# hpc4cmb/flacarray

Measured on AMD Instinct MI355X. Metric: Msamples/s encode+decode, 4096ch x 1Msamp int32, higher is better.
Workload: dtype int32

## Files before the change

### flacarray_amd/csrc/encode_fused.hpp

```cpp
#pragma once
#include "encode_kernels.hpp"
#include "quantize_kernels.hpp"

namespace fa {

constexpr int kFSmpWords = 65 * 32;
#ifndef FA_F_SCANW
#define FA_F_SCANW 4
#endif
#ifndef FA_F_RING
#define FA_F_RING 1024
#endif
constexpr int kFRingWords = FA_F_RING;
constexpr int kFRingMask = kFRingWords - 1;
constexpr int kFRingBlocks = kFRingWords / 64;
constexpr int kFRowBlocks = 12;
static_assert(kFRingBlocks - kFRowBlocks - 1 >= 1, "the ring must hold the longest row and a partial block beside what waits to be flushed");
constexpr int kFWaveWords = kFSmpWords + kFRingWords + 4 + 16;
constexpr int kFWaves = 4;
constexpr int kFCrcSlice = 1024;
constexpr int kFCrcXpow = 520;
#ifndef FA_F_SLEEP
#define FA_F_SLEEP 8
#endif
#ifndef FA_F_WBATCH
#define FA_F_WBATCH 4
#endif
#ifndef FA_F_CEIL
#define FA_F_CEIL 1
#endif
#ifndef FA_F_BFLY_N
#define FA_F_BFLY_N 1
#endif
#ifndef FA_F_SHLEV
#define FA_F_SHLEV 1
#endif
#ifndef FA_F_SHLEV_MAXMLO
#define FA_F_SHLEV_MAXMLO 12
#endif
#ifndef FA_F_SHPOLL
#define FA_F_SHPOLL 256
#endif
#ifndef FA_F_SHSLEEP
#define FA_F_SHSLEEP 4
#endif
#ifndef FA_F_PARKN
#define FA_F_PARKN 32
#endif
#ifndef FA_F_PARKBLK
#define FA_F_PARKBLK 1
#endif
#ifndef FA_F_PARK
#define FA_F_PARK 1
#endif
// ... 12 lines not shown
    double escale_full;
    const float* win;
    const uint4* hdr;
    uint8_t* blob;
    int64_t capacity;
    int64_t hb;
    uint32_t* frame_bytes;
    int64_t* frame_abs;
    FrameInfo* info;
    uint32_t* ticket;
    uint32_t* size_pub;
    unsigned long long* off_pub;
    int64_t* total;
    int* err;
    const uint16_t* crc_tab;
    unsigned long long* stamps;
    int64_t* starts;
    int64_t* nbytes;
};

__device__ __forceinline__ int fsmp_unit(int c1, int u) { return 32 * c1 + 4 * (u ^ (c1 & 7)); }
__device__ __forceinline__ int fsmp_idx(int s) {
    const int c1 = (s >> 5) + 1;
    return fsmp_unit(c1, (s >> 2) & 7) + (s & 3);
}

__device__ __forceinline__ int lane_id_opaque() {
    int l;
    asm volatile("v_mbcnt_lo_u32_b32 %0, -1, 0\n\tv_mbcnt_hi_u32_b32 %0, -1, %0" : "=v"(l));
    return l;
}
__device__ __forceinline__ int rice_fold(int r) { return (int)(((uint32_t)r << 1) ^ (uint32_t)(r >> 31)); }
__device__ __forceinline__ int dpp_wave_shr1(int old, int v) { return __builtin_amdgcn_update_dpp(old, v, 0x138, 0xF, 0xF, false); }

__device__ __forceinline__ uint16_t crc16_mulmod(uint16_t a, uint16_t b) {
    uint32_t r = 0;
#pragma unroll
    for (int i = 15; i >= 0; --i) {
        r = (r << 1) ^ ((r & 0x8000u) ? 0x18005u : 0u);
        if ((b >> i) & 1) r ^= a;
    }
    return (uint16_t)r;
}

template <typename T>
__device__ __forceinline__ T lb_load(const T* p) { return __hip_atomic_load(p, __ATOMIC_RELAXED, __HIP_MEMORY_SCOPE_AGENT); }

struct SplitRiceSearch {
    int pred_order, pmax, lane;
    uint32_t TA, TB, S, n, pb, SC, best;
    int M, p, k, bpo, kb;
    bool slot;
    __device__ __forceinline__ void start(uint32_t ta, uint32_t tb, int pred_order_, int pmax_, int lane_) {
        pred_order = pred_order_; pmax = pmax_; lane = lane_;
        TA = wave_incl_scan_u32(ta);
        TB = wave_incl_scan_u32(tb);
    }
    __device__ __forceinline__ void gather() {
        M = (2 << pmax) - 1;
        const int Lp = M - lane;
        slot = (Lp >= 1);
        const int po = slot ? (31 - __clz(Lp)) : 0;
        p = lane - (M + 1 - (2 << po));
        const uint32_t psz = 4096u >> po;
        const int cpp = 128 >> po;
        const bool inB = (po > 0) && (p >= (1 << (po - 1)));
// ... 996 lines not shown
        a.info[g].shift = (int32_t)(uint32_t)__builtin_amdgcn_s_memrealtime();
        __builtin_amdgcn_s_waitcnt(0);
    }
#endif
    if (lane_w == 0) {
        __hip_atomic_store(a.size_pub + gu, 0x80000000u | total_bytes, __ATOMIC_RELAXED, __HIP_MEMORY_SCOPE_AGENT);
        a.frame_bytes[g] = total_bytes;
    }
    (void)F;
#ifndef FA_TIMELINE
    if (lane_w == 0 && a.info) {
        FrameInfo fi;
        fi.type = type;
        fi.order = (type >= 2) ? order : 0;
        fi.porder = (type >= 2) ? porder : 0;
        fi.wasted = wasted;
        fi.shift = (type == 3) ? shift : 0;
        fi.precision = (type == 3) ? precision : 0;
        fi.nbytes = (int32_t)total_bytes;
        fi.blocksize = bs;
        a.info[g] = fi;
    }
#endif

#ifdef FA_F_ANALYSIS_ONLY
    if (lane_w == 0) a.frame_abs[g] = g * (int64_t)kSlotBytes + (s + 1) * a.hb;
    return;
#endif
    kpar[lane_w] = (uint8_t)kbest;
    for (int i = lane_w; i < kFRingWords; i += 64) ring[i] = 0;
    if (lane_w == 0) ring[kFRingWords] = 0;
    lds_fence();
    uint32_t pos = 0;
    uint32_t blocks_flushed = 0;
    uint8_t* dst = nullptr;
    bool dropped = false, have_dst = false;
    uint32_t crc_t = 0;

    auto put_bits = [&](uint32_t P, uint32_t val, uint32_t nb) __attribute__((always_inline)) {
        const uint32_t off = P & 31u;
        const uint64_t X = (uint64_t)val << (64u - nb - off);
        const uint32_t a0 = (P >> 3) & (uint32_t)(4 * kFRingWords - 4);
        atomicOr(reinterpret_cast<uint32_t*>(reinterpret_cast<char*>(ring) + a0), (uint32_t)(X >> 32));
        atomicOr(reinterpret_cast<uint32_t*>(reinterpret_cast<char*>(ring) + a0 + 4), (uint32_t)X);
    };
    auto put_code = [&](uint32_t P, uint32_t u, uint32_t shl) __attribute__((always_inline)) {
        const uint32_t vL = (u << shl) | 0x80000000u;
        uint32_t wi;
        asm("v_bfe_u32 %0, %1, 5, %2" : "=v"(wi) : "v"(P), "n"(__builtin_ctz((unsigned)kFRingWords)));
        uint32_t* const w = ring + wi;
        atomicOr(w, __builtin_amdgcn_alignbit(0u, vL, P));
        atomicOr(w + 1, __builtin_amdgcn_alignbit(vL, 0u, P));
    };
    unsigned long long off_word = 0;
    auto lb_issue = [&]() __attribute__((always_inline)) {
#ifndef FA_F_NOLB
        off_word = lb_load(a.off_pub + gu);
#endif
    };
    auto lb_resolve = [&]() __attribute__((always_inline)) {
        uint32_t spins = 0;
        bool fail = false;
#ifdef FA_TIMELINE
        const uint32_t tl_req_ = (uint32_t)__builtin_amdgcn_s_memrealtime();
#endif
#ifdef FA_F_NOLB
        off_word = (unsigned long long)(g * (int64_t)kSlotBytes + (s + 1) * a.hb);
#else
        while (off_word == 0) {
            __builtin_amdgcn_s_sleep(FA_F_SLEEP);
            if (++spins > kLbSpinLimit) { fail = true; break; }
            off_word = lb_load(a.off_pub + gu);
        }
#endif
#ifdef FA_TIMELINE
        if (lane_w == 0 && a.info) {
            a.info[g].precision = (int32_t)tl_req_;
            a.info[g].blocksize = (int32_t)(uint32_t)__builtin_amdgcn_s_memrealtime();
        }
#endif
#ifdef FA_STAMPS
        st_[3] += spins;
#endif
        const int64_t off = (int64_t)(((uint64_t)(uint32_t)__builtin_amdgcn_readfirstlane((int)(uint32_t)(off_word >> 32)) << 32) |
                                      (uint32_t)__builtin_amdgcn_readfirstlane((int)(uint32_t)off_word));
        fail = __builtin_amdgcn_readfirstlane((int)fail) != 0;
        if (fail || off < 0 || off + (int64_t)total_bytes > a.capacity) {
            if (lane_w == 0) atomicOr(a.err, fail ? 2 : 1);
            dropped = true;
        } else {
            dst = a.blob + off;
            if (lane_w == 0) a.frame_abs[g] = off;
        }
        have_dst = true;
    };
    auto crc_word = [&](uint32_t wv) __attribute__((always_inline)) {
        const uint32_t w = wv ^ (crc_t << 16);
        const uint32_t t0 = crc_s[w >> 24], t1 = crc_s[256 + ((w >> 16) & 255u)], t2 = crc_s[512 + ((w >> 8) & 255u)], t3 = crc_s[768 + (w & 255u)];
        uint32_t x01;
        asm("v_xor_b32 %0, %1, %2" : "=v"(x01) : "v"(t0), "v"(t1));
        asm("v_bitop3_b32 %0, %1, %2, %3 bitop3:0x96" : "=v"(crc_t) : "v"(x01), "v"(t2), "v"(t3));
    };
    uint32_t carry = 0;
    auto emit_word = [&](uint32_t m, uint32_t Q) __attribute__((always_inline)) {
        const uint32_t sh = (uint32_t)(reinterpret_cast<uintptr_t>(dst) & 3u);
        const uint32_t P = (uint32_t)dpp_wave_shr1((int)carry, (int)Q);
        carry = (uint32_t)__builtin_amdgcn_readlane((int)Q, 63);
        const uint32_t V = __builtin_amdgcn_alignbit(P, Q, 8u * sh);
        const int lo = (int)(4u * m) - (int)sh;
        if (lo >= 0 && (uint32_t)lo + 4u <= total_bytes) {
            *reinterpret_cast<uint32_t*>(dst + lo) = __builtin_bswap32(V);
        } else {
#pragma unroll
            for (int i = 0; i < 4; ++i) {
                const int b = lo + i;
                if (b >= 0 && (uint32_t)b < total_bytes) dst[b] = (uint8_t)(V >> (24 - 8 * i));
            }
        }
    };
    auto emit_block = [&](uint32_t blk, uint32_t Q) __attribute__((always_inline)) {
        const uint32_t sh = (uint32_t)(reinterpret_cast<uintptr_t>(dst) & 3u);
        const uint32_t P = (uint32_t)dpp_wave_shr1((int)carry, (int)Q);
        carry = (uint32_t)__builtin_amdgcn_readlane((int)Q, 63);
        const uint32_t V = __builtin_amdgcn_alignbit(P, Q, 8u * sh);
        *reinterpret_cast<uint32_t*>(dst - sh + 256u * blk + 4u * (uint32_t)lane_w) = __builtin_bswap32(V);
    };
#if FA_F_PARKBLK
    uint32_t park[FA_F_PARKN];
#endif
    uint32_t n_parked = 0;
    auto take_block = [&](uint32_t blk) __attribute__((always_inline)) {
        const uint32_t wi = (blk * 64 + lane_w) & kFRingMask;
        uint32_t wv = ring[wi];
        ring[wi] = 0;
        if (__builtin_expect((blk & (uint32_t)(kFRingBlocks - 1)) == 0, 0)) {
            if (lane_w == 0) { wv |= ring[kFRingWords]; ring[kFRingWords] = 0; }
        }
        return wv;
    };
    auto flush_blocks = [&](uint32_t row_bits, bool final_call) __attribute__((always_inline)) {
        const uint32_t done = (uint32_t)__builtin_amdgcn_readfirstlane((int)(pos >> 11));
        blocks_flushed = (uint32_t)__builtin_amdgcn_readfirstlane((int)blocks_flushed);
        const uint32_t hi_blk = (uint32_t)__builtin_amdgcn_readfirstlane((int)((pos + row_bits) >> 11));
        if (!final_call && hi_blk - blocks_flushed < (uint32_t)kFRingBlocks) return;
#ifdef FA_STAMPS
        const unsigned long long tq0_ = fa_memtime();
#endif
        if (!have_dst) {
#if FA_F_PARKBLK
            if (!final_call && off_word == 0) {
                off_word = lb_load(a.off_pub + gu);
                n_parked = (uint32_t)__builtin_amdgcn_readfirstlane((int)n_parked);
                while (blocks_flushed < done && n_parked < (uint32_t)FA_F_PARKN) {
                    const uint32_t wv = take_block(blocks_flushed);
                    crc_word(wv);
                    park[n_parked] = wv;
                    n_parked++;
                    blocks_flushed++;
                }
                if (hi_blk - blocks_flushed < (uint32_t)kFRingBlocks) {
#ifdef FA_STAMPS
                    st_[14] += fa_memtime() - tq0_;
#endif
                    return;
                }
            }
#endif
            lb_resolve();
        }
#ifdef FA_STAMPS
        st_[14] += fa_memtime() - tq0_;
#endif
#if FA_F_PARKBLK
        n_parked = (uint32_t)__builtin_amdgcn_readfirstlane((int)n_parked);
        if (__builtin_expect(n_parked != 0, 0)) {
            if (!dropped) {
                emit_word((uint32_t)lane_w, park[0]);
                for (uint32_t i = 1; i < n_parked; ++i) emit_block(i, park[i]);
            }
            n_parked = 0;
        }
#endif
        if (__builtin_expect(blocks_flushed == 0 && done > 0, 0)) {
            const uint32_t wv = take_block(0);
            crc_word(wv);
            if (!dropped) emit_word((uint32_t)lane_w, wv);
            blocks_flushed = 1;
            __builtin_amdgcn_sched_barrier(0);
        }
        while (blocks_flushed < done) {
            const uint32_t wv = take_block(blocks_flushed);
            crc_word(wv);
            if (!dropped) emit_block(blocks_flushed, wv);
            blocks_flushed++;
        }
    };

#if FA_F_PARKBLK
#pragma unroll
    for (int i = 0; i < FA_F_PARKN; ++i) asm volatile("" : "=v"(park[i]));
#endif
    lb_issue();
    {
        const int tc = (type == 0) ? 0x00 : (type == 1) ? 0x01 : (type == 2) ? (0x08 | order) : (0x20 | (order - 1));
        const uint32_t smask = (bps == 32) ? 0xffffffffu : ((1u << bps) - 1u);
        const int nwarm = (type == 0) ? 1 : (type >= 2) ? order : 0;
        constexpr int kWarmLanes = (MLO > 4) ? MLO : 4;
        constexpr int kL_warm = 6, kL_lpc = kL_warm + kWarmLanes, kL_coef = kL_lpc + 1, kL_rice = kL_coef + MLO;
        static_assert(kL_rice < 64, "preamble fields must fit the wave");
        uint32_t fv = 0, fnb = 0;
        if (lane_w == 0) { fv = fhe.x; fnb = 32; }
        else if (lane_w == 1) { fv = fhe.y; fnb = (fhe.w >> 8) & 0xFFu; }
        else if (lane_w == 2) { fv = fhe.z & 0xFFFFu; fnb = (fhe.w >> 16) & 0xFFu; }
        else if (lane_w == 3) { fv = fhe.z >> 16; fnb = fhe.w >> 24; }
        else if (lane_w == 4) { fv = ((fhe.w & 0xFFu) << 8) | (uint32_t)((tc << 1) | (wasted ? 1 : 0)); fnb = 16; }
        else if (lane_w == 5) { if (wasted) { fv = 1; fnb = (uint32_t)wasted; } }
        else if (lane_w < kL_lpc) {
            if (lane_w - kL_warm < nwarm) {
                fv = (uint32_t)smp[fsmp_idx(lane_w - kL_warm)] & smask;
                fnb = (uint32_t)bps;
            }
        }
        else if (lane_w == kL_lpc) { if (type == 3) { fv = ((uint32_t)(precision - 1) << 5) | (uint32_t)shift; fnb = 9; } }
        else if (lane_w < kL_rice) {
            if (type == 3 && lane_w - kL_coef < order) {
                int32_t q = 0;
#pragma unroll
                for (int j = 0; j < MLO; ++j) q = (lane_w - kL_coef == j) ? qkeep[j] : q;
                fv = (uint32_t)q & ((1u << precision) - 1u);
                fnb = (uint32_t)precision;
            }
        }
        else if (lane_w == kL_rice) { if (type >= 2) { fv = ((rice2 ? 1u : 0u) << 4) | (uint32_t)porder; fnb = 6; } }
// ... 74 lines not shown
#pragma unroll
                for (int e = 0; e < 8; ++e) {
                    if constexpr (FIRST) {
                        if (q[e] != 0xffffffffu) {
                            if (gb + (uint32_t)e == pstart) put_bits(p, k, (uint32_t)plen);
                            put_bits(p + q[e], onek | (us[e] & mask), kp1);
                            p += q[e] + kp1;
                        }
                    } else {
                        put_code(p + q[e], us[e], 31u - k);
                        p += q[e] + kp1;
                    }
                }
                if constexpr (!FIRST) {
                    if (newp) put_bits(p0, k, (uint32_t)plen);
                }
                pos += total;
            };
            row8(std::true_type{}, 0);
#pragma unroll 1
            for (int j = 1; j < 8; ++j) {
                if (j == 4) store_b();
                row8(std::false_type{}, j);
            }
        }
    }

    FA_STAMP(11);
    flush_blocks(0u, true);
    if (!have_dst) lb_resolve();
    FA_STAMP(13);
    {
        const uint32_t nwords = (total_bytes + 3u) >> 2;
        uint32_t last_end = 256u * blocks_flushed - 256u + 4u * (uint32_t)lane_w + 4u;
        bool any = blocks_flushed > 0;
        for (uint32_t w0 = blocks_flushed * 64; w0 < nwords; w0 += 64) {
            const uint32_t wl = w0 + lane_w;
            if (4u * wl < L) {
                uint32_t wv = ring[wl & kFRingMask];
                if ((wl & kFRingMask) == 0) wv |= ring[kFRingWords];
                crc_word(wv);
                last_end = 4u * wl + 4u;
                any = true;
            }
        }
        uint32_t contrib = 0;
        if (any) {
            const int after = (int)L - (int)last_end;
            contrib = crc16_mulmod((uint16_t)crc_t, a.crc_tab[kFCrcSlice + after + 3]);
        }
        contrib ^= (uint32_t)xchg_i32<0>((int)contrib);
        contrib ^= (uint32_t)xchg_i32<1>((int)contrib);
        contrib ^= (uint32_t)xchg_i32<2>((int)contrib);
        contrib ^= (uint32_t)xchg_i32<3>((int)contrib);
        contrib ^= (uint32_t)xchg_i32<4>((int)contrib);
        const uint32_t crc = ((uint32_t)__builtin_amdgcn_readlane((int)contrib, 0) ^ (uint32_t)__builtin_amdgcn_readlane((int)contrib, 32)) & 0xFFFFu;
        lds_fence();
        if (lane_w == 0) put_bits(8u * L, crc, 16);
        lds_fence();
        if (!dropped) {
            for (uint32_t w0 = blocks_flushed * 64; w0 <= nwords; w0 += 64) {
                const uint32_t wl = w0 + lane_w;
                uint32_t wv = 0;
                if (wl < nwords) {
                    wv = ring[wl & kFRingMask];
                    if ((wl & kFRingMask) == 0) wv |= ring[kFRingWords];
                }
                emit_word(wl, wv);
            }
        }
    }
    FA_STAMP(12);
#ifdef FA_STAMPS
    if (lane_w == 0 && a.stamps && (blockIdx.x % 61u) == 0) {
        uint32_t xcc;
        asm volatile("s_getreg_b32 %0, hwreg(HW_REG_XCC_ID)" : "=s"(xcc));
        xcc &= 7u;
        unsigned long long life = 0;
        for (int i_ = 0; i_ < 13; ++i_) life += st_[i_];
        atomicAdd(&a.stamps[32 + 4 * xcc], 1ULL);
        atomicAdd(&a.stamps[33 + 4 * xcc], st_[14]);
        atomicAdd(&a.stamps[34 + 4 * xcc], life);
        unsigned long long prep = 0;
        for (int i_ = 0; i_ < 10; ++i_) prep += st_[i_];
        atomicAdd(&a.stamps[35 + 4 * xcc], prep);
    }
#endif
    FA_STAMP_FLUSH;
}

__global__ __launch_bounds__(256) void fused_finish_kernel(uint8_t* __restrict__ out, const int64_t* __restrict__ frame_abs,
                                                           const uint32_t* __restrict__ frame_bytes, int64_t n_stream, int64_t nframes,
                                                           int64_t stream_size, int32_t B, int32_t tail_bs, int32_t nch, int64_t hb,
                                                           int64_t* __restrict__ starts, int64_t* __restrict__ nbytes,
// ... 118 lines not shown
```

### flacarray_amd/csrc/flacarray_hip.hip

```cpp
#include <hip/hip_runtime.h>

#include <cmath>
#include <cstdio>
#include <cstdlib>
#include <cstring>
#include <algorithm>
#include <atomic>
#include <condition_variable>
#include <functional>
#include <map>
#include <memory>
#include <mutex>
#include <new>
#include <thread>
#include <vector>

#include <sys/mman.h>
#include <time.h>
#include <unistd.h>

#include "../../include/flacarray_hip.h"
#include "decode_kernels.hpp"
#ifndef FA_SPLIT_UNITS
#define FA_HAVE_K5_LAUNCHERS 1
// ... 3 lines not shown
#include "encode_placed.hpp"
#include "decode_latency.hpp"
#include "quantize_kernels.hpp"
#include "verify_kernels.hpp"
#include "std_kernels.hpp"
#include "splice_kernels.hpp"
#include "md5_kernels.hpp"
#include "reduce_kernels.hpp"
#include "scrub_kernels.hpp"
#include "reindex_kernels.hpp"
#include "window_kernels.hpp"
#include "join_kernels.hpp"

namespace {

using namespace fa;

#define FA_HIP_TRY(expr)                                                                          \
    do {                                                                                          \
        hipError_t e_ = (expr);                                                                   \
        if (e_ != hipSuccess) {                                                                   \
            std::fprintf(stderr, "flacarray_hip: %s failed: %s\n", #expr, hipGetErrorString(e_)); \
            return FA_ERROR_DEVICE;                                                               \
        }                                                                                         \
    } while (0)

constexpr int kProfPairs = 6;
constexpr int kScratchSlots = 23;
struct DeviceState {
    std::recursive_mutex api_mu;
    std::map<int, float*> windows;
    uint16_t* crc_tab = nullptr;
    uint16_t* crc_tab_fused = nullptr;
    void* scratch[kScratchSlots] = {};
    size_t scratch_bytes[kScratchSlots] = {};
    uint64_t scratch_epoch = 1;
    std::vector<uint4> h_hdr;
    int64_t c_nf = -1;
    int c_B = 0, c_tail = 0, c_nch = 0;
    void* c_dp = nullptr;
    uint64_t c_epoch = 0;
    bool stamps_zeroed = false;
    int64_t std_plan_key[2] = {-1, -1};
    uint64_t std_plan_epoch = 0;
    hipStream_t feed_stream = nullptr;
    void* pin = nullptr;
    void* pin_dev = nullptr;
    bool pin_tried = false;
    hipStream_t verify_stream = nullptr;
    hipEvent_t verify_ev[2] = {nullptr, nullptr};
    bool verify_tried = false;
    hipEvent_t ev[2 * kProfPairs];
    bool ev_ready = false;
    bool ev_set[kProfPairs] = {false, false, false, false, false, false};
};
std::mutex g_mu;
std::map<int, std::unique_ptr<DeviceState>> g_dev;
std::atomic<bool> g_prof{false};
std::atomic<bool> g_verify{false};
std::atomic<bool> g_encode_verify{false};
std::atomic<bool> g_encode_md5{false};

DeviceState* dev_state() {
    int d = 0;
    if (hipGetDevice(&d) != hipSuccess) return nullptr;
    std::lock_guard<std::mutex> lk(g_mu);
// ... 80 lines not shown

int get_crc_tab(const uint16_t** out) {
    DeviceState* st = dev_state();
    if (!st) return FA_ERROR_DEVICE;
    if (!st->crc_tab) {
        std::vector<uint16_t> t((size_t)kCrcTabWords);
        auto feed = [](uint16_t c, uint8_t v) { return crc16_byte(c, v); };
        for (int k = 0; k < 4; ++k)
            for (int v = 0; v < 256; ++v) {
                uint16_t c = 0;
                for (int b = 0; b < 4; ++b) c = feed(c, (uint8_t)(b == k ? v : 0));
                t[(size_t)(k * 256 + v)] = c;
            }
        for (int v = 0; v < 256; ++v) {
            uint16_t hi = (uint16_t)(v << 8), lo = (uint16_t)v;
            for (int b = 0; b < 256; ++b) { hi = feed(hi, 0); lo = feed(lo, 0); }
            t[(size_t)(1024 + v)] = hi;
            t[(size_t)(1280 + v)] = lo;
        }
        uint16_t xp = 1;
        for (int n = 0; n < 512; ++n) {
            t[(size_t)(1536 + n)] = xp;
            xp = feed(xp, 0);
        }
        uint16_t* d = nullptr;
        FA_HIP_TRY(hipMalloc(&d, sizeof(uint16_t) * (size_t)kCrcTabWords));
        FA_HIP_TRY(hipMemcpy(d, t.data(), sizeof(uint16_t) * (size_t)kCrcTabWords, hipMemcpyHostToDevice));
        st->crc_tab = d;
    }
    *out = st->crc_tab;
    return FA_ERROR_NONE;
}

int get_crc_tab_fused(const uint16_t** out) {
    DeviceState* st = dev_state();
    if (!st) return FA_ERROR_DEVICE;
    if (!st->crc_tab_fused) {
        std::vector<uint16_t> t((size_t)(kFCrcSlice + kFCrcXpow));
        auto mulx8 = [](uint16_t c) { return crc16_byte(c, 0); };
        auto mulmod = [](uint16_t a, uint16_t b) {
            uint32_t r = 0;
            for (int i = 15; i >= 0; --i) {
                r = (r << 1) ^ ((r & 0x8000u) ? 0x18005u : 0u);
                if ((b >> i) & 1) r ^= a;
            }
            return (uint16_t)r;
        };
        int ord = 0;
        for (uint16_t c = 1;;) { c = mulx8(c); ++ord; if (c == 1) break; }
        auto xpow8 = [&](long k) {
            k %= ord;
            if (k < 0) k += ord;
            uint16_t c = 1;
            for (long i = 0; i < k; ++i) c = mulx8(c);
            return c;
        };
        const uint16_t x2016 = xpow8(252);
        for (int k = 0; k < 4; ++k)
            for (int v = 0; v < 256; ++v) {
                uint16_t c = 0;
                for (int b = 0; b < 4; ++b) c = crc16_byte(c, (uint8_t)(b == k ? v : 0));
                t[(size_t)(k * 256 + v)] = mulmod(c, x2016);
            }
        {
            uint16_t c = xpow8(-255);
            for (int i = 0; i < kFCrcXpow; ++i) { t[(size_t)(kFCrcSlice + i)] = c; c = mulx8(c); }
        }
        uint16_t* d = nullptr;
        FA_HIP_TRY(hipMalloc(&d, sizeof(uint16_t) * t.size()));
        FA_HIP_TRY(hipMemcpy(d, t.data(), sizeof(uint16_t) * t.size(), hipMemcpyHostToDevice));
        st->crc_tab_fused = d;
    }
    *out = st->crc_tab_fused;
    return FA_ERROR_NONE;
}

inline size_t align_up(size_t v, size_t a) { return (v + a - 1) / a * a; }

struct FramePlan {
    LevelParams P;
    uint32_t level;
    int nch;
    int64_t n_stream, stream_size;
    int64_t B, nf, F, hb;
    int tail_bs;
    int64_t slot_stride;
    int64_t capacity;
    int32_t pmax_full, pmax_tail;
    double escale_full, escale_tail;
};

int make_frame_plan(int64_t n_stream, int64_t stream_size, uint32_t level, int nch, FramePlan* fp) {
    if (level > 8) return FA_ERROR_INVALID_LEVEL;
    if (n_stream <= 0) return FA_ERROR_ZERO_NSTREAM;
    if (stream_size <= 0) return FA_ERROR_ZERO_STREAMSIZE;
    fp->P = level_params(level);
    fp->level = level; fp->nch = nch; fp->n_stream = n_stream; fp->stream_size = stream_size;
    fp->B = fp->P.blocksize;
    fp->nf = (stream_size + fp->B - 1) / fp->B;
    fp->tail_bs = (int)(stream_size - (fp->nf - 1) * fp->B);
    if (18 * fp->nf >= (1 << 24)) return FA_ERROR_ENCODE_PROCESS;
    if (fp->nf > 0x7fffffffLL / n_stream) return FA_ERROR_ENCODE_PROCESS;
    fp->F = n_stream * fp->nf;
    fp->hb = stream_header_bytes(fp->nf);
    fp->slot_stride = (int64_t)kSlotBytes * nch;
    fp->capacity = fp->F * fp->slot_stride + n_stream * fp->hb;
// ... 95 lines not shown
        l.off_tzero = o;  o = align_up(o + (size_t)fp.n_stream * 8, 256);
    }
    l.total = o;
    return l;
}


struct PlacedLayout {
    PublishBlock pub;
    size_t off_slots, total;
};

constexpr int64_t kPlacedBelowFrames = 4096;
int64_t placed_grid(int64_t F) {
    int64_t g = kPlacedGrid;
    if (const char* e = std::getenv("FLACARRAY_HIP_PLACED_GRID")) {
        const long v = std::atol(e);
        if (v >= 64 && v <= 16384) g = v;
    }
    return std::min<int64_t>(g, F) + 1;
}

PlacedLayout placed_layout(const FramePlan& fp) {
    PlacedLayout l;
    size_t o = lay_publish_block(fp.F, &l.pub);
    l.off_slots = o;  o = align_up(o + (size_t)placed_grid(fp.F) * 2 * (size_t)fp.slot_stride + 256 * (size_t)(FA_PG_GROUP) + 256, 256);
    l.total = o;
    return l;
}

int run_verify(const DecodeArgs& a, int* d_err, int* h_err, hipStream_t st, int verify) {
    if (!(verify < 0 ? g_verify.load() : verify != 0)) return FA_ERROR_NONE;
    const uint16_t* tab = nullptr;
    int rc = get_crc_tab_fused(&tab);
    if (rc) return rc;
    hipLaunchKernelGGL(verify_crc16_kernel, dim3((unsigned)((a.n_tasks + 3) / 4)), dim3(256), 0, st, a, tab);
    FA_HIP_TRY(hipMemcpyAsync(h_err, d_err, 16, hipMemcpyDeviceToHost, st));
    FA_HIP_TRY(hipStreamSynchronize(st));
    return FA_ERROR_NONE;
}

bool run_verify_beside_begin(hipStream_t st) {
    DeviceState* ds = dev_state();
    if (!ds) return false;
    if (!ds->verify_tried) {
        ds->verify_tried = true;
        hipStream_t vs = nullptr;
        int least = 0, greatest = 0;
        (void)hipDeviceGetStreamPriorityRange(&least, &greatest);
        const char* pe = std::getenv("FLACARRAY_HIP_VERIFY_PRIO");
        int prio = least;
        if (pe && pe[0] == 'h') prio = greatest;
        else if (pe && pe[0] == 'n') prio = (least + greatest) / 2;
        if (hipStreamCreateWithPriority(&vs, hipStreamNonBlocking, prio) == hipSuccess) {
            if (hipEventCreateWithFlags(&ds->verify_ev[0], hipEventDisableTiming) == hipSuccess &&
                hipEventCreateWithFlags(&ds->verify_ev[1], hipEventDisableTiming) == hipSuccess) {
                ds->verify_stream = vs;
            } else {
                (void)hipStreamDestroy(vs);
            }
        }
        if (!ds->verify_stream) (void)hipGetLastError();
    }
    if (!ds->verify_stream) return false;
    if (hipEventRecord(ds->verify_ev[0], st) != hipSuccess) return false;
    return hipStreamWaitEvent(ds->verify_stream, ds->verify_ev[0], 0) == hipSuccess;
}
bool run_verify_beside_launch(const DecodeArgs& a, hipStream_t st) {
    DeviceState* ds = dev_state();
    const uint16_t* tab = nullptr;
    if (!ds || !ds->verify_stream || get_crc_tab_fused(&tab)) return false;
    hipLaunchKernelGGL(verify_crc16_kernel, dim3((unsigned)((a.n_tasks + 3) / 4)), dim3(256), 0, ds->verify_stream, a, tab);
    (void)hipEventRecord(ds->verify_ev[1], ds->verify_stream);
    (void)hipStreamWaitEvent(st, ds->verify_ev[1], 0);
    return true;
}

constexpr size_t kPinBytes = 512u << 10;
bool pinned_landing(void** host, void** dev) {
    DeviceState* ds = dev_state();
    if (!ds) return false;
    if (!ds->pin_tried) {
        ds->pin_tried = true;
        void* h = nullptr;
        void* d = nullptr;
        if (hipHostMalloc(&h, kPinBytes + 64, hipHostMallocDefault) == hipSuccess) {
            if (hipHostGetDevicePointer(&d, h, 0) == hipSuccess) { ds->pin = h; ds->pin_dev = d; }
            else (void)hipHostFree(h);
        } else {
            (void)hipGetLastError();
        }
    }
    *host = ds->pin;
    *dev = ds->pin_dev;
    return ds->pin != nullptr;
}

bool latency_allowed(int64_t n_tasks) {
    const char* e = std::getenv("FLACARRAY_HIP_LATENCY");
    if (e && e[0] == '0') return false;
    if (e && e[0] == '1') return n_tasks <= 65535;
    return n_tasks <= 4096;
}

// ... 744 lines not shown
    const FusedLayout pl = fused_layout(fp);
    const int64_t n_stream = fp.n_stream, stream_size = fp.stream_size;
    if (!d_workspace || workspace_bytes < single_pass_need(fp)) return FA_ERROR_ALLOC;
    if (!d_bytes || capacity_bytes < n_stream * fp.hb + 64) return FA_ERROR_ALLOC;
    hipStream_t st = reinterpret_cast<hipStream_t>(stream);
    char* ws = reinterpret_cast<char*>(d_workspace);
    prof_begin(3, st);
    int* d_nanflag = reinterpret_cast<int*>(ws + pl.pub.off_ticket + 12);
    FA_HIP_TRY(hipMemsetAsync(ws + pl.pub.off_zero, 0, pl.pub.zero_bytes, st));
    if (f32) {
        const int64_t cps = (stream_size + kRangeChunk - 1) / kRangeChunk;
        void* pp = nullptr;
        int rcp = get_scratch(10, (size_t)n_stream * (size_t)cps * 8 + 256, &pp);
        if (rcp) return rcp;
        float* pmin = reinterpret_cast<float*>(pp);
        float* pmax = pmin + n_stream * cps;
        prof_begin(5, st);
        hipLaunchKernelGGL(float32_range_kernel, dim3((unsigned)(n_stream * cps)), dim3(256), 0, st, reinterpret_cast<const float*>(d_data),
                           stream_size, cps, pmin, pmax, d_nanflag);
        hipLaunchKernelGGL(float32_params_kernel, dim3((unsigned)((n_stream + 255) / 256)), dim3(256), 0, st, pmin, pmax, n_stream, cps,
                           d_quanta, d_offsets, d_gains);
        prof_end(5, st);
    }
    FusedArgs a;
    std::memset(&a, 0, sizeof a);
    a.data = reinterpret_cast<const int32_t*>(d_data); a.f_offsets = d_offsets; a.f_gains = d_gains; a.n_stream = n_stream; a.stream_size = stream_size; a.nframes = fp.nf; a.total_frames = fp.F;
    a.max_lpc_order = fp.P.max_lpc_order; a.max_porder = fp.P.max_porder; a.precision = fp.P.qlp_precision;
    a.pmax_full = fp.pmax_full;
    a.escale_full = fp.escale_full;
    a.tail_bs = fp.tail_bs;
    const bool tails = (fp.tail_bs != kMaxBlock);
    int rc = get_window(kMaxBlock, &a.win);
    if (rc) return rc;
    rc = get_crc_tab_fused(&a.crc_tab);
    if (rc) return rc;
    rc = frame_header_table(ds_, fp, st, &a.hdr);
    if (rc) return rc;
    a.blob = d_bytes; a.capacity = capacity_bytes; a.hb = fp.hb;
    point_into_publish_block(pl.pub, ws, &a);
    a.info = reinterpret_cast<FrameInfo*>(d_info);
    a.stamps = stamps_scratch(ds_);
    if (tails) {
        EncodeArgs t;
        rc = fill_encode_args(fp, a.data, reinterpret_cast<uint8_t*>(ws + pl.off_tslots), a.frame_bytes, d_info, &t);
        if (rc) return rc;
        t.hdr = a.hdr;
        t.tail_only = 1;
        launch_encode_for(t, 1, n_stream, st);
        launch_fused_tail_publish(st, a.frame_bytes, a.size_pub, n_stream, fp.nf);
    }
    prof_begin(0, st);
    launch_fused_encode(st, a, f32);
    prof_end(0, st);
    PublishBack back = {0, 0, 0};
    rc = read_publish_back(a, st, &back);
    if (rc) return rc;
    if (tails) {
        uint32_t* tb = reinterpret_cast<uint32_t*>(ws + pl.off_tbytes);
        int64_t* toff = reinterpret_cast<int64_t*>(ws + pl.off_toff);
        int64_t* tzero = reinterpret_cast<int64_t*>(ws + pl.off_tzero);
        launch_fused_tail_prep(st, a.off_pub, a.frame_bytes, n_stream, fp.nf, a.frame_abs, tb, toff, tzero);
        const uint16_t* crc5 = nullptr;
        rc = get_crc_tab(&crc5);
        if (rc) return rc;
        int64_t nblk = (n_stream + 3) / 4;
        if (nblk > 32768) nblk = 32768;
        launch_compact_frames(st, nblk, reinterpret_cast<const uint8_t*>(ws + pl.off_tslots), tb, toff, tzero, 1, n_stream, crc5, d_bytes, kSlotBytes);
// ... 866 lines not shown
struct ScrubTables {
    const unsigned char* bytes = nullptr;
    StreamMeta* meta = nullptr;
    int64_t* ftab = nullptr;
    int* err = nullptr;
    int64_t nf = 0;
};

static int scrub_run(const unsigned char* d_bytes, int64_t n_bytes, const int64_t* d_starts, const int64_t* d_nbytes, int64_t n_stream,
                     int64_t stream_size, int channels, int64_t block_size, unsigned char* d_status, hipStream_t st, ScrubTables* tb) {
    if (n_stream <= 0) return FA_ERROR_ZERO_NSTREAM;
    if (stream_size <= 0) return FA_ERROR_DECODE_STREAMSIZE;
    if (channels != 1 && channels != 2) return FA_ERROR_CONVERT_TYPE;
    if (block_size < 1 || block_size > 65535) return FA_ERROR_DECODE_INIT;
    if (n_bytes < 0 || !d_starts || !d_nbytes || !d_status || (n_bytes > 0 && !d_bytes)) return FA_ERROR_DECODE_INIT;
    const int32_t B = (int32_t)block_size;
    const int64_t nf = (stream_size + B - 1) / B;
    if (nf > (int64_t)0x7fffffff * 4 / n_stream) return FA_ERROR_DECODE_SAMPLE_RANGE;
    const int64_t nt = n_stream * nf;
    if (reinterpret_cast<uintptr_t>(d_bytes) & 15) {
        void* al = nullptr;
        int rc0 = get_scratch(17, (size_t)n_bytes + 256, &al);
        if (rc0) return rc0;
        FA_HIP_TRY(hipMemcpyAsync(al, d_bytes, (size_t)n_bytes, hipMemcpyDeviceToDevice, st));
        d_bytes = reinterpret_cast<const unsigned char*>(al);
    }
    const size_t meta_bytes = align_up((size_t)n_stream * sizeof(StreamMeta), 256);
    const size_t flag_bytes = align_up((size_t)n_stream, 256);
    void *p = nullptr, *pt = nullptr;
    int rc = get_scratch(18, meta_bytes + flag_bytes + 256, &p);
    if (rc) return rc;
    if ((rc = get_scratch(19, (size_t)nt * 8 + 256, &pt))) return rc;
    const uint16_t* tab = nullptr;
    if ((rc = get_crc_tab_fused(&tab))) return rc;
    StreamMeta* d_meta = reinterpret_cast<StreamMeta*>(p);
    uint8_t* d_located = reinterpret_cast<uint8_t*>(p) + meta_bytes;
    int* d_err = reinterpret_cast<int*>(reinterpret_cast<char*>(p) + meta_bytes + flag_bytes);
    int64_t* d_ftab = reinterpret_cast<int64_t*>(pt);
    FA_HIP_TRY(hipMemsetAsync(d_err, 0, 256, st));
    hipLaunchKernelGGL(scrub_streams_kernel, dim3((unsigned)((n_stream + 255) / 256)), dim3(256), 0, st, d_bytes, d_starts, d_nbytes, n_stream, nf,
                       n_bytes, B, (int32_t)channels, d_meta, d_located);
    hipLaunchKernelGGL(scrub_table_kernel, dim3((unsigned)((nt + 255) / 256)), dim3(256), 0, st, d_bytes, d_meta, d_located, n_stream, nf, B, d_ftab);
    hipLaunchKernelGGL(frame_status_kernel, dim3((unsigned)((nt + 3) / 4)), dim3(256), 0, st, d_bytes, n_bytes, d_meta, d_ftab, n_stream, nf, B,
                       stream_size, (int32_t)channels, tab, d_status);
    FA_HIP_TRY(hipGetLastError());
    if (tb) { tb->bytes = d_bytes; tb->meta = d_meta; tb->ftab = d_ftab; tb->err = d_err; tb->nf = nf; }
    return FA_ERROR_NONE;
}

int fa_frame_status_device(const unsigned char* d_bytes, int64_t n_bytes, const int64_t* d_starts, const int64_t* d_nbytes, int64_t n_stream,
                           int64_t stream_size, int channels, int64_t block_size, unsigned char* d_status, void* stream) {
    FA_API_LOCK;
    hipStream_t st = reinterpret_cast<hipStream_t>(stream);
    const int rc = scrub_run(d_bytes, n_bytes, d_starts, d_nbytes, n_stream, stream_size, channels, block_size, d_status, st, nullptr);
    if (rc) return rc;
    FA_HIP_TRY(hipStreamSynchronize(st));
    return FA_ERROR_NONE;
}

int fa_fill_ranges_device(void* d_out, int elem_bytes, int64_t n_ranges, const int64_t* d_off, const int64_t* d_count, const void* fill_value,
                          void* stream) {
    FA_API_LOCK;
    if (elem_bytes != 4 && elem_bytes != 8) return FA_ERROR_CONVERT_TYPE;
    if (n_ranges < 0 || !fill_value) return FA_ERROR_DECODE_SAMPLE_RANGE;
    if (n_ranges == 0) return FA_ERROR_NONE;
    if (!d_out || !d_off || !d_count) return FA_ERROR_DECODE_INIT;
    hipStream_t st = reinterpret_cast<hipStream_t>(stream);
// ... 1159 lines not shown
```

Before: 219,500.

## Flush ring in 128-word units with two interleaved CRC chains

The fused encoder's bitstream flush now drains the LDS ring 128 words per step instead of 64. Each lane carries two independent CRC16 chains (one per half-unit), and the sliced CRC table is parameterised by unit size, with a separate table kept for the verify/check kernels. The readlane carry is replaced with a DPP rotate, and the CRC top-half xor uses an SDWA instruction. This is meant to halve loop iterations and expose more instruction-level parallelism in the LDS loads and table lookups, at the cost of more registers for the parked words and a more complex tail CRC combine.

```diff
diff --git a/flacarray_amd/csrc/encode_fused.hpp b/flacarray_amd/csrc/encode_fused.hpp
--- a/flacarray_amd/csrc/encode_fused.hpp
+++ b/flacarray_amd/csrc/encode_fused.hpp
@@ -13,13 +13,16 @@
 #endif
 constexpr int kFRingWords = FA_F_RING;
 constexpr int kFRingMask = kFRingWords - 1;
-constexpr int kFRingBlocks = kFRingWords / 64;
-constexpr int kFRowBlocks = 12;
-static_assert(kFRingBlocks - kFRowBlocks - 1 >= 1, "the ring must hold the longest row and a partial block beside what waits to be flushed");
+constexpr int kFUnitWords = 128;
+constexpr int kFRingBlocks = kFRingWords / kFUnitWords;
+constexpr int kFRowBlocks = 6;
+static_assert(kFRingBlocks - kFRowBlocks - 1 >= 1, "the ring must hold the longest row and a partial unit beside what waits to be flushed");
 constexpr int kFWaveWords = kFSmpWords + kFRingWords + 4 + 16;
 constexpr int kFWaves = 4;
 constexpr int kFCrcSlice = 1024;
-constexpr int kFCrcXpow = 520;
+constexpr int kFCrcUnit = 4 * kFUnitWords;
+constexpr int kFCrcXpow = 2 * kFCrcUnit + 8;
+constexpr int kCheckCrcUnit = 256;
 #ifndef FA_F_SLEEP
 #define FA_F_SLEEP 8
 #endif
@@ -98,6 +101,7 @@
 }
 __device__ __forceinline__ int rice_fold(int r) { return (int)(((uint32_t)r << 1) ^ (uint32_t)(r >> 31)); }
 __device__ __forceinline__ int dpp_wave_shr1(int old, int v) { return __builtin_amdgcn_update_dpp(old, v, 0x138, 0xF, 0xF, false); }
+__device__ __forceinline__ int dpp_wave_ror1(int v) { return __builtin_amdgcn_mov_dpp(v, 0x13C, 0xF, 0xF, false); }
 
 __device__ __forceinline__ uint16_t crc16_mulmod(uint16_t a, uint16_t b) {
     uint32_t r = 0;
@@ -1160,10 +1164,10 @@
     if (lane_w == 0) ring[kFRingWords] = 0;
     lds_fence();
     uint32_t pos = 0;
-    uint32_t blocks_flushed = 0;
+    uint32_t units_flushed = 0;
     uint8_t* dst = nullptr;
     bool dropped = false, have_dst = false;
-    uint32_t crc_t = 0;
+    uint32_t crc_t = 0, crc_u = 0;
 
     auto put_bits = [&](uint32_t P, uint32_t val, uint32_t nb) __attribute__((always_inline)) {
         const uint32_t off = P & 31u;
@@ -1222,18 +1226,33 @@
         }
         have_dst = true;
     };
-    auto crc_word = [&](uint32_t wv) __attribute__((always_inline)) {
-        const uint32_t w = wv ^ (crc_t << 16);
-        const uint32_t t0 = crc_s[w >> 24], t1 = crc_s[256 + ((w >> 16) & 255u)], t2 = crc_s[512 + ((w >> 8) & 255u)], t3 = crc_s[768 + (w & 255u)];
+    auto crc_top = [&](uint32_t state, uint32_t wv) __attribute__((always_inline)) {
+        uint32_t h;
+        asm("v_xor_b32_sdwa %0, %1, %2 dst_sel:DWORD dst_unused:UNUSED_PAD src0_sel:DWORD src1_sel:WORD_1" : "=v"(h) : "v"(state), "v"(wv));
+        return h;
+    };
+    auto crc_word = [&](uint32_t& state, uint32_t wv) __attribute__((always_inline)) {
+        const uint32_t h = crc_top(state, wv);
+        const uint32_t t0 = crc_s[(h >> 8) & 255u], t1 = crc_s[256 + (h & 255u)], t2 = crc_s[512 + ((wv >> 8) & 255u)], t3 = crc_s[768 + (wv & 255u)];
         uint32_t x01;
         asm("v_xor_b32 %0, %1, %2" : "=v"(x01) : "v"(t0), "v"(t1));
+        asm("v_bitop3_b32 %0, %1, %2, %3 bitop3:0x96" : "=v"(state) : "v"(x01), "v"(t2), "v"(t3));
+    };
+    auto crc_unit = [&](uint32_t wv0, uint32_t wv1) __attribute__((always_inline)) {
+        const uint32_t h = crc_top(crc_t, wv0), g = crc_top(crc_u, wv1);
+        const uint32_t t0 = crc_s[(h >> 8) & 255u], t1 = crc_s[256 + (h & 255u)], t2 = crc_s[512 + ((wv0 >> 8) & 255u)], t3 = crc_s[768 + (wv0 & 255u)];
+        const uint32_t u0 = crc_s[(g >> 8) & 255u], u1 = crc_s[256 + (g & 255u)], u2 = crc_s[512 + ((wv1 >> 8) & 255u)], u3 = crc_s[768 + (wv1 & 255u)];
+        uint32_t x01, y01;
+        asm("v_xor_b32 %0, %1, %2" : "=v"(x01) : "v"(t0), "v"(t1));
+        asm("v_xor_b32 %0, %1, %2" : "=v"(y01) : "v"(u0), "v"(u1));
         asm("v_bitop3_b32 %0, %1, %2, %3 bitop3:0x96" : "=v"(crc_t) : "v"(x01), "v"(t2), "v"(t3));
+        asm("v_bitop3_b32 %0, %1, %2, %3 bitop3:0x96" : "=v"(crc_u) : "v"(y01), "v"(u2), "v"(u3));
     };
     uint32_t carry = 0;
     auto emit_word = [&](uint32_t m, uint32_t Q) __attribute__((always_inline)) {
         const uint32_t sh = (uint32_t)(reinterpret_cast<uintptr_t>(dst) & 3u);
         const uint32_t P = (uint32_t)dpp_wave_shr1((int)carry, (int)Q);
-        carry = (uint32_t)__builtin_amdgcn_readlane((int)Q, 63);
+        carry = (uint32_t)dpp_wave_ror1((int)Q);
         const uint32_t V = __builtin_amdgcn_alignbit(P, Q, 8u * sh);
         const int lo = (int)(4u * m) - (int)sh;
         if (lo >= 0 && (uint32_t)lo + 4u <= total_bytes) {
@@ -1249,28 +1268,43 @@
     auto emit_block = [&](uint32_t blk, uint32_t Q) __attribute__((always_inline)) {
         const uint32_t sh = (uint32_t)(reinterpret_cast<uintptr_t>(dst) & 3u);
         const uint32_t P = (uint32_t)dpp_wave_shr1((int)carry, (int)Q);
-        carry = (uint32_t)__builtin_amdgcn_readlane((int)Q, 63);
+        carry = (uint32_t)dpp_wave_ror1((int)Q);
         const uint32_t V = __builtin_amdgcn_alignbit(P, Q, 8u * sh);
         *reinterpret_cast<uint32_t*>(dst - sh + 256u * blk + 4u * (uint32_t)lane_w) = __builtin_bswap32(V);
     };
+    auto emit_unit = [&](uint32_t u, uint32_t Q0, uint32_t Q1) __attribute__((always_inline)) {
+        const uint32_t sh = (uint32_t)(reinterpret_cast<uintptr_t>(dst) & 3u);
+        const uint32_t R0 = (uint32_t)dpp_wave_ror1((int)Q0), R1 = (uint32_t)dpp_wave_ror1((int)Q1);
+        const uint32_t P0 = (lane_w == 0) ? carry : R0, P1 = (lane_w == 0) ? R0 : R1;
+        carry = R1;
+        const uint32_t V0 = __builtin_amdgcn_alignbit(P0, Q0, 8u * sh), V1 = __builtin_amdgcn_alignbit(P1, Q1, 8u * sh);
+        uint32_t* const d = reinterpret_cast<uint32_t*>(dst - sh + 512u * u + 4u * (uint32_t)lane_w);
+        d[0] = __builtin_bswap32(V0);
+        d[64] = __builtin_bswap32(V1);
+    };
+    auto emit_first_unit = [&](uint32_t Q0, uint32_t Q1) __attribute__((always_inline)) {
+        emit_word((uint32_t)lane_w, Q0);
+        emit_block(1u, Q1);
+    };
 #if FA_F_PARKBLK
-    uint32_t park[FA_F_PARKN];
+    uint32_t park0[FA_F_PARKN / 2], park1[FA_F_PARKN / 2];
 #endif
     uint32_t n_parked = 0;
-    auto take_block = [&](uint32_t blk) __attribute__((always_inline)) {
-        const uint32_t wi = (blk * 64 + lane_w) & kFRingMask;
-        uint32_t wv = ring[wi];
-        ring[wi] = 0;
-        if (__builtin_expect((blk & (uint32_t)(kFRingBlocks - 1)) == 0, 0)) {
-            if (lane_w == 0) { wv |= ring[kFRingWords]; ring[kFRingWords] = 0; }
-        }
-        return wv;
+    auto take_unit = [&](uint32_t u, uint32_t& w0, uint32_t& w1) __attribute__((always_inline)) {
+        uint32_t* const r = ring + ((u * (uint32_t)kFUnitWords + (uint32_t)lane_w) & (uint32_t)kFRingMask);
+        w0 = r[0];
+        w1 = r[64];
+        r[0] = 0;
+        r[64] = 0;
+        if (__builtin_expect((u & (uint32_t)(kFRingBlocks - 1)) == 0, 0)) {
+            if (lane_w == 0) { w0 |= ring[kFRingWords]; ring[kFRingWords] = 0; }
+        }
     };
     auto flush_blocks = [&](uint32_t row_bits, bool final_call) __attribute__((always_inline)) {
-        const uint32_t done = (uint32_t)__builtin_amdgcn_readfirstlane((int)(pos >> 11));
-        blocks_flushed = (uint32_t)__builtin_amdgcn_readfirstlane((int)blocks_flushed);
-        const uint32_t hi_blk = (uint32_t)__builtin_amdgcn_readfirstlane((int)((pos + row_bits) >> 11));
-        if (!final_call && hi_blk - blocks_flushed < (uint32_t)kFRingBlocks) return;
+        const uint32_t done = (uint32_t)__builtin_amdgcn_readfirstlane((int)(pos >> 12));
+        units_flushed = (uint32_t)__builtin_amdgcn_readfirstlane((int)units_flushed);
+        const uint32_t hi_unit = (uint32_t)__builtin_amdgcn_readfirstlane((int)((pos + row_bits) >> 12));
+        if (!final_call && hi_unit - units_flushed < (uint32_t)kFRingBlocks) return;
 #ifdef FA_STAMPS
         const unsigned long long tq0_ = fa_memtime();
 #endif
@@ -1279,14 +1313,16 @@
             if (!final_call && off_word == 0) {
                 off_word = lb_load(a.off_pub + gu);
                 n_parked = (uint32_t)__builtin_amdgcn_readfirstlane((int)n_parked);
-                while (blocks_flushed < done && n_parked < (uint32_t)FA_F_PARKN) {
-                    const uint32_t wv = take_block(blocks_flushed);
-                    crc_word(wv);
-                    park[n_parked] = wv;
+                while (units_flushed < done && n_parked < (uint32_t)(FA_F_PARKN / 2)) {
+                    uint32_t w0, w1;
+                    take_unit(units_flushed, w0, w1);
+                    crc_unit(w0, w1);
+                    park0[n_parked] = w0;
+                    park1[n_parked] = w1;
                     n_parked++;
-                    blocks_flushed++;
-                }
-                if (hi_blk - blocks_flushed < (uint32_t)kFRingBlocks) {
+                    units_flushed++;
+                }
+                if (hi_unit - units_flushed < (uint32_t)kFRingBlocks) {
 #ifdef FA_STAMPS
                     st_[14] += fa_memtime() - tq0_;
 #endif
@@ -1303,30 +1339,32 @@
         n_parked = (uint32_t)__builtin_amdgcn_readfirstlane((int)n_parked);
         if (__builtin_expect(n_parked != 0, 0)) {
             if (!dropped) {
-                emit_word((uint32_t)lane_w, park[0]);
-                for (uint32_t i = 1; i < n_parked; ++i) emit_block(i, park[i]);
+                emit_first_unit(park0[0], park1[0]);
+                for (uint32_t i = 1; i < n_parked; ++i) emit_unit(i, park0[i], park1[i]);
             }
             n_parked = 0;
         }
 #endif
-        if (__builtin_expect(blocks_flushed == 0 && done > 0, 0)) {
-            const uint32_t wv = take_block(0);
-            crc_word(wv);
-            if (!dropped) emit_word((uint32_t)lane_w, wv);
-            blocks_flushed = 1;
+        if (__builtin_expect(units_flushed == 0 && done > 0, 0)) {
+            uint32_t w0, w1;
+            take_unit(0, w0, w1);
+            crc_unit(w0, w1);
+            if (!dropped) emit_first_unit(w0, w1);
+            units_flushed = 1;
             __builtin_amdgcn_sched_barrier(0);
         }
-        while (blocks_flushed < done) {
-            const uint32_t wv = take_block(blocks_flushed);
-            crc_word(wv);
-            if (!dropped) emit_block(blocks_flushed, wv);
-            blocks_flushed++;
+        while (units_flushed < done) {
+            uint32_t w0, w1;
+            take_unit(units_flushed, w0, w1);
+            crc_unit(w0, w1);
+            if (!dropped) emit_unit(units_flushed, w0, w1);
+            units_flushed++;
         }
     };
 
 #if FA_F_PARKBLK
 #pragma unroll
-    for (int i = 0; i < FA_F_PARKN; ++i) asm volatile("" : "=v"(park[i]));
+    for (int i = 0; i < FA_F_PARKN / 2; ++i) asm volatile("" : "=v"(park0[i]), "=v"(park1[i]));
 #endif
     lb_issue();
     {
@@ -1467,23 +1505,24 @@
     FA_STAMP(13);
     {
         const uint32_t nwords = (total_bytes + 3u) >> 2;
-        uint32_t last_end = 256u * blocks_flushed - 256u + 4u * (uint32_t)lane_w + 4u;
-        bool any = blocks_flushed > 0;
-        for (uint32_t w0 = blocks_flushed * 64; w0 < nwords; w0 += 64) {
-            const uint32_t wl = w0 + lane_w;
-            if (4u * wl < L) {
-                uint32_t wv = ring[wl & kFRingMask];
-                if ((wl & kFRingMask) == 0) wv |= ring[kFRingWords];
-                crc_word(wv);
-                last_end = 4u * wl + 4u;
-                any = true;
-            }
+        const uint32_t wl0 = units_flushed * (uint32_t)kFUnitWords + (uint32_t)lane_w, wl1 = wl0 + 64u;
+        uint32_t end0 = 4u * wl0 - (uint32_t)kFCrcUnit + 4u, end1 = 4u * wl1 - (uint32_t)kFCrcUnit + 4u;
+        bool any0 = units_flushed > 0, any1 = any0;
+        if (4u * wl0 < L) {
+            uint32_t wv = ring[wl0 & kFRingMask];
+            if ((wl0 & kFRingMask) == 0) wv |= ring[kFRingWords];
+            crc_word(crc_t, wv);
+            end0 = 4u * wl0 + 4u;
+            any0 = true;
+        }
+        if (4u * wl1 < L) {
+            crc_word(crc_u, ring[wl1 & kFRingMask]);
+            end1 = 4u * wl1 + 4u;
+            any1 = true;
         }
         uint32_t contrib = 0;
-        if (any) {
-            const int after = (int)L - (int)last_end;
-            contrib = crc16_mulmod((uint16_t)crc_t, a.crc_tab[kFCrcSlice + after + 3]);
-        }
+        if (any0) contrib = crc16_mulmod((uint16_t)crc_t, a.crc_tab[kFCrcSlice + (int)L - (int)end0 + 3]);
+        if (any1) contrib ^= crc16_mulmod((uint16_t)crc_u, a.crc_tab[kFCrcSlice + (int)L - (int)end1 + 3]);
         contrib ^= (uint32_t)xchg_i32<0>((int)contrib);
         contrib ^= (uint32_t)xchg_i32<1>((int)contrib);
         contrib ^= (uint32_t)xchg_i32<2>((int)contrib);
@@ -1494,7 +1533,7 @@
         if (lane_w == 0) put_bits(8u * L, crc, 16);
         lds_fence();
         if (!dropped) {
-            for (uint32_t w0 = blocks_flushed * 64; w0 <= nwords; w0 += 64) {
+            for (uint32_t w0 = units_flushed * (uint32_t)kFUnitWords; w0 <= nwords; w0 += 64) {
                 const uint32_t wl = w0 + lane_w;
                 uint32_t wv = 0;
                 if (wl < nwords) {
diff --git a/flacarray_amd/csrc/flacarray_hip.hip b/flacarray_amd/csrc/flacarray_hip.hip
--- a/flacarray_amd/csrc/flacarray_hip.hip
+++ b/flacarray_amd/csrc/flacarray_hip.hip
@@ -59,6 +59,7 @@
     std::map<int, float*> windows;
     uint16_t* crc_tab = nullptr;
     uint16_t* crc_tab_fused = nullptr;
+    uint16_t* crc_tab_check = nullptr;
     void* scratch[kScratchSlots] = {};
     size_t scratch_bytes[kScratchSlots] = {};
     uint64_t scratch_epoch = 1;
@@ -205,11 +206,13 @@
     return FA_ERROR_NONE;
 }
 
-int get_crc_tab_fused(const uint16_t** out) {
+int get_crc_tab_fused(const uint16_t** out, int unit) {
     DeviceState* st = dev_state();
     if (!st) return FA_ERROR_DEVICE;
-    if (!st->crc_tab_fused) {
-        std::vector<uint16_t> t((size_t)(kFCrcSlice + kFCrcXpow));
+    uint16_t*& slot = (unit == kFCrcUnit) ? st->crc_tab_fused : st->crc_tab_check;
+    if (!slot) {
+        const int nxpow = 2 * unit + 8;
+        std::vector<uint16_t> t((size_t)(kFCrcSlice + nxpow));
         auto mulx8 = [](uint16_t c) { return crc16_byte(c, 0); };
         auto mulmod = [](uint16_t a, uint16_t b) {
             uint32_t r = 0;
@@ -228,23 +231,23 @@
             for (long i = 0; i < k; ++i) c = mulx8(c);
             return c;
         };
-        const uint16_t x2016 = xpow8(252);
+        const uint16_t xadv = xpow8(unit - 4);
         for (int k = 0; k < 4; ++k)
             for (int v = 0; v < 256; ++v) {
                 uint16_t c = 0;
                 for (int b = 0; b < 4; ++b) c = crc16_byte(c, (uint8_t)(b == k ? v : 0));
-                t[(size_t)(k * 256 + v)] = mulmod(c, x2016);
+                t[(size_t)(k * 256 + v)] = mulmod(c, xadv);
             }
         {
-            uint16_t c = xpow8(-255);
-            for (int i = 0; i < kFCrcXpow; ++i) { t[(size_t)(kFCrcSlice + i)] = c; c = mulx8(c); }
+            uint16_t c = xpow8(-(unit - 1));
+            for (int i = 0; i < nxpow; ++i) { t[(size_t)(kFCrcSlice + i)] = c; c = mulx8(c); }
         }
         uint16_t* d = nullptr;
         FA_HIP_TRY(hipMalloc(&d, sizeof(uint16_t) * t.size()));
         FA_HIP_TRY(hipMemcpy(d, t.data(), sizeof(uint16_t) * t.size(), hipMemcpyHostToDevice));
-        st->crc_tab_fused = d;
-    }
-    *out = st->crc_tab_fused;
+        slot = d;
+    }
+    *out = slot;
     return FA_ERROR_NONE;
 }
 
@@ -406,7 +409,7 @@
 int run_verify(const DecodeArgs& a, int* d_err, int* h_err, hipStream_t st, int verify) {
     if (!(verify < 0 ? g_verify.load() : verify != 0)) return FA_ERROR_NONE;
     const uint16_t* tab = nullptr;
-    int rc = get_crc_tab_fused(&tab);
+    int rc = get_crc_tab_fused(&tab, kCheckCrcUnit);
     if (rc) return rc;
     hipLaunchKernelGGL(verify_crc16_kernel, dim3((unsigned)((a.n_tasks + 3) / 4)), dim3(256), 0, st, a, tab);
     FA_HIP_TRY(hipMemcpyAsync(h_err, d_err, 16, hipMemcpyDeviceToHost, st));
@@ -443,7 +446,7 @@
 bool run_verify_beside_launch(const DecodeArgs& a, hipStream_t st) {
     DeviceState* ds = dev_state();
     const uint16_t* tab = nullptr;
-    if (!ds || !ds->verify_stream || get_crc_tab_fused(&tab)) return false;
+    if (!ds || !ds->verify_stream || get_crc_tab_fused(&tab, kCheckCrcUnit)) return false;
     hipLaunchKernelGGL(verify_crc16_kernel, dim3((unsigned)((a.n_tasks + 3) / 4)), dim3(256), 0, ds->verify_stream, a, tab);
     (void)hipEventRecord(ds->verify_ev[1], ds->verify_stream);
     (void)hipStreamWaitEvent(st, ds->verify_ev[1], 0);
@@ -1254,7 +1257,7 @@
     const bool tails = (fp.tail_bs != kMaxBlock);
     int rc = get_window(kMaxBlock, &a.win);
     if (rc) return rc;
-    rc = get_crc_tab_fused(&a.crc_tab);
+    rc = get_crc_tab_fused(&a.crc_tab, kFCrcUnit);
     if (rc) return rc;
     rc = frame_header_table(ds_, fp, st, &a.hdr);
     if (rc) return rc;
@@ -2187,7 +2190,7 @@
     if (rc) return rc;
     if ((rc = get_scratch(19, (size_t)nt * 8 + 256, &pt))) return rc;
     const uint16_t* tab = nullptr;
-    if ((rc = get_crc_tab_fused(&tab))) return rc;
+    if ((rc = get_crc_tab_fused(&tab, kCheckCrcUnit))) return rc;
     StreamMeta* d_meta = reinterpret_cast<StreamMeta*>(p);
     uint8_t* d_located = reinterpret_cast<uint8_t*>(p) + meta_bytes;
     int* d_err = reinterpret_cast<int*>(reinterpret_cast<char*>(p) + meta_bytes + flag_bytes);
```

Result: no change. 220,700, median of 3 (+0.6%).
